# ActiveVisionLab/gaussctrl

Measured on AMD Instinct MI355X. Metric: edited views/sec @512x512 (ControlNet denoise + splat render+bwd), higher is better.
Workload: dtype bf16

## Files before the change

gaussctrl_amd/csrc/dn_gemm.hip:

```cpp
#include "dn_gemm_kernels.h"

namespace {

int choose_splits(int64_t blocks, int nk)
{
    if (blocks >= 128 || nk < 32) return 1;
    int s = (int)((448 + blocks - 1) / blocks);
    if (s > nk / 8) s = nk / 8;
    if (s > 16) s = 16;
    return s < 2 ? 1 : s;
}

int choose_mt(int64_t M, int64_t N, int ntw, bool forced)
{
    const int64_t nbn = (N + 32 * ntw - 1) / (32 * ntw);
    if (((M + 127) / 128) * nbn < 96 && !forced) return 0;
    int best = 2;
    int64_t best_cost = -1;
    for (int mt = 2; mt <= 4; ++mt) {
        const int64_t tiles = ((M + 64 * mt - 1) / (64 * mt)) * nbn;
        const int64_t cost = ((tiles + 255) / 256) * (mt + 1);
        if (best_cost < 0 || cost < best_cost || (cost == best_cost && mt == 4)) { best = mt; best_cost = cost; }
    }
    return best;
// ... 4 lines not shown
    int64_t r = total_wgs / 8 < 1 ? 1 : total_wgs / 8;
    if (r > conc) r = conc;
    const int64_t tiles = nbm * nbn;
    if (r >= tiles) return 0;
    const int64_t ca = conv ? bm : 9 * bm, cw = 9 * bn;
    int best = 0;
    int64_t best_cost = -1;
    for (int64_t pw = nbn; pw >= 1; --pw) {
        const int64_t per = nbm * pw;
        const int64_t cols = std::min<int64_t>(nbn, pw * ((r + per - 1) / per)), rows = std::min<int64_t>(nbm, (r + pw - 1) / pw);
        const int64_t cost = rows * ca + cols * cw;
        if (best_cost < 0 || cost < best_cost) { best = pw == nbn ? 0 : (int)pw; best_cost = cost; }
    }
    return best;
}

int pw_of(const gc_gemm_desc *d, int64_t nbm, int64_t nbn, int64_t total_wgs, int conc, int64_t bm, int64_t bn)
{
    const int f = (d->kernel_variant >> 16) & 0xff;
    if (f) return f - 1;
    return choose_pw(nbm, nbn, total_wgs, conc, bm, bn, d->mode == 1);
}

void plan(const gc_gemm_desc *d, int *ntw, int *splits, int *tps)
{
    *ntw = (d->N % 160 == 0 && d->N % 128 != 0 && !d->geglu) ? 5 : 4;
    if (d->softmax_keys > 0) *ntw = 5;
    const int bn = 32 * *ntw;
    const int64_t Msel = d->plan_rows > 0 ? d->plan_rows : d->M;
    const int64_t blocks = ((Msel + BM - 1) / BM) * ((d->N + bn - 1) / bn);
    const int nk = (int)((d->K + BK - 1) / BK);
    *splits = (d->geglu || d->w_set_rows > 0 || d->softmax_keys > 0) ? 1 : choose_splits(blocks, nk);
    *tps = (nk + *splits - 1) / *splits;
    *splits = (nk + *tps - 1) / *tps;
}


struct SelQ { int ntw, mt, splits, tps; };
void select_fp8(const gc_gemm_desc *d, SelQ *o, bool assume_ws)
{
    const int force_mt = d->kernel_variant & 7;
    o->ntw = (d->N % 160 == 0 && d->N % 128 != 0 && !d->geglu) ? 5 : 4;
    int mt = force_mt ? force_mt : choose_mt(d->M, d->N, o->ntw, true);
    if (o->ntw == 5) mt = 2; else if (mt > 3) mt = 3;
    if (mt < 2) mt = 2;
    const int nkq = (int)(d->K / 128);
    o->splits = 1; o->tps = nkq;
    const bool plain = !d->geglu && !d->out_t && !d->out_fp8 && !d->out_f32 && d->out && !d->ln_row_stats && !d->out_row_stats && !d->out_group_stats && d->act == 0;
    const int64_t Msel = d->plan_rows > 0 ? d->plan_rows : d->M;
    const int64_t nbn = (d->N + 32 * o->ntw - 1) / (32 * o->ntw), tiles = ((Msel + 127) / 128) * nbn;
    if (plain && !force_mt && !(d->kernel_variant & 0x40) && tiles <= 128 && nkq >= 16) {
        int s = (int)std::min<int64_t>(tiles < 96 ? (256 + tiles - 1) / tiles : 256 / tiles, nkq / 8);
        if (s > 16) s = 16;
        if (s >= 2 && (assume_ws || (d->workspace && d->workspace_bytes >= sizeof(float) * (size_t)s * (size_t)d->M * (size_t)d->N))) {
            mt = 2; o->tps = (nkq + s - 1) / s; o->splits = (nkq + o->tps - 1) / o->tps;
        }
    }
    o->mt = mt;
}
}

extern "C" size_t gc_dn_gemm_workspace_bytes(const gc_gemm_desc *d)
{
    if (!d || d->M <= 0 || d->N <= 0 || d->K <= 0) return 0;
    if (d->fp8) {
        if (d->K % 128 != 0) return 0;
        SelQ q;
        select_fp8(d, &q, true);
        return q.splits > 1 ? sizeof(float) * (size_t)q.splits * (size_t)d->M * (size_t)d->N : 0;
    }
    int ntw, splits, tps;
    plan(d, &ntw, &splits, &tps);
    return splits > 1 ? sizeof(float) * (size_t)splits * (size_t)d->M * (size_t)d->N : 0;
}

namespace {
int ln_lean_kind(const gc_gemm_desc *d)
{
    if ((d->kernel_variant & 0x800) || d->fp8 || d->mode != 0 || d->K % 64 != 0 || d->out_group_stats || d->out_chan_parts || d->N < 4) return 0;
    if (d->out_row_stats && !d->ln_row_stats)
        return (!d->geglu && d->act == 0 && !d->out_f32 && !d->out_t && d->out && (!d->rowvec || d->rows_per_batch >= 256)) ? 1 : 0;
    if (d->ln_row_stats && !d->out_row_stats) return d->softmax_keys > 0 ? 3 : 2;
    return 0;
}
struct Sel { int mode, ntw, splits, tps, mt8; };
int select(const gc_gemm_desc *d, Sel *o, bool want_parts)
{
    int mode = 0;
    if (d->mode == 1) mode = (d->Cin % 64 == 0) ? 2 : 1;
    int ntw, splits, tps;
    plan(d, &ntw, &splits, &tps);
    if (splits > 1 && (!d->workspace || d->workspace_bytes < sizeof(float) * (size_t)splits * (size_t)d->M * (size_t)d->N)) {
        splits = 1; tps = (int)((d->K + BK - 1) / BK);
    }
    const int bn = 32 * ntw;
    const int64_t nbn = (d->N + bn - 1) / bn;
    const int nk_host = (int)((d->K + BK - 1) / BK);
    const int kv = d->kernel_variant;
    const int force_mt = kv & 7;
    const int use8 = (kv & 0x10) ? 0 : ((kv & 0x20) ? 2 : 1);
    const int convsplit = (kv & 0x40) ? 0 : ((kv & 0x80) ? 1 : 2);
    o->mode = mode; o->ntw = ntw; o->splits = splits; o->tps = tps; o->mt8 = 0;
    if (use8 && d->zeros) {
        const int64_t Msel = d->plan_rows > 0 ? d->plan_rows : d->M;
        int mt = force_mt ? force_mt : choose_mt(Msel, d->N, ntw, use8 == 2);
        if (mt && !force_mt && Msel != d->M) mt = choose_mt(d->M, d->N, ntw, true);
        const int64_t tiles8 = ((Msel + 127) / 128) * nbn;
        const bool small = tiles8 < 96;
        if (!mt && mode == 0 && !force_mt) mt = 2;
        if (mode == 0 && !force_mt && ntw == 4 && d->K % 64 == 0 && !d->geglu && !d->out_t && !(kv & 0x100) &&
            (!(d->ln_row_stats || d->out_row_stats || d->out_group_stats) || ln_lean_kind(d)) && !want_parts) {
            const int64_t t1 = ((d->M + 63) / 64) * nbn, t2 = ((d->M + 127) / 128) * nbn;
            if (mt == 2 && t2 <= 256 && t1 <= 512 && t1 > 128 && nk_host <= 24) mt = 1;
        }
        if (d->w_set_rows > 0 && mt) {
            int pick = 0;
            const int cand[5] = {mt, 4, 3, 2, (ntw == 4 && d->softmax_keys == 0) ? 1 : 2};
            for (int c = 0; c < 5 && !pick; ++c) if (d->w_set_rows % (64 * cand[c]) == 0) pick = cand[c];
            mt = pick ? pick : mt;
        }
        const bool want_split = !force_mt && use8 != 2 && !d->geglu && d->w_set_rows == 0 && d->softmax_keys == 0 && d->workspace && tiles8 <= 128 && (mode == 0 ? (!small || nk_host >= 24) : (convsplit >= (small ? 2 : 1)));
        int s8 = 1, tps8 = nk_host;
        if (want_split) {
            const int smt = (kv >> 24) & 7;
            const bool img8 = mode != 0 && !small && d->Ho * d->Wo <= 64 && Msel % 256 == 0;
            const int mts = (smt >= 2 && smt <= 4) ? smt : (img8 ? 4 : ((mode != 0 && !small) ? 3 : 2));
            const int64_t tiles_s = ((Msel + 64 * mts - 1) / (64 * mts)) * nbn;
            s8 = (int)std::min<int64_t>(std::max<int64_t>(256 / tiles_s, 2), nk_host / 12);
            if (s8 >= 2 && d->workspace_bytes >= sizeof(float) * (size_t)s8 * (size_t)d->M * (size_t)d->N) {
                mt = mts; tps8 = (nk_host + s8 - 1) / s8; s8 = (nk_host + tps8 - 1) / tps8;
            } else s8 = 1;
        }
        if (splits > 1 && s8 == 1 && !force_mt && use8 != 2) mt = 0;
        if (mt) { o->mt8 = mt; o->splits = s8; o->tps = tps8; }
    }
    return 0;
}
}

extern "C" int gc_dn_gemm_row_stat_slots(const gc_gemm_desc *d)
{
    if (!d || d->M <= 0 || d->N <= 0 || d->K <= 0) return 0;
    if (d->fp8) { const int ntw = (d->N % 160 == 0 && d->N % 128 != 0) ? 5 : 4; return (int)((d->N + 16 * ntw - 1) / (16 * ntw)); }
    Sel sel;
    select(d, &sel, false);
    return sel.splits > 1 ? (int)((d->N / 4 + 63) / 64) : (int)((d->N + 16 * sel.ntw - 1) / (16 * sel.ntw));
}

namespace {
void chan_parts_layout(const gc_gemm_desc *d, const Sel &sel, int64_t *rows, int *nslab, int *col_tile)
{
    *rows = 0; *nslab = 0; *col_tile = 0;
    const int64_t rpb = d->rows_per_batch;
    if (d->fp8) {
        SelQ q;
        select_fp8(d, &q, false);
        if (d->K % 128 != 0 || rpb < 256 || rpb % 32 != 0 || d->M % rpb != 0 || d->gn_groups < 1 || d->N % d->gn_groups != 0) return;
        const int64_t cpg = d->N / d->gn_groups;
        if (q.splits > 1) {
            if (cpg > 64) return;
            *rows = CS_RB; *nslab = (int)(rpb / CS_RB); *col_tile = 64;
            return;
        }
        const bool lean = d->mode == 1 && !d->upsample && !d->geglu && !d->out_t && !d->out_fp8 && !d->out_f32 && d->out && d->act == 0 &&
                          !d->ln_row_stats && !d->out_row_stats && !d->out_group_stats;
        const int64_t bm = 64 * q.mt;
        if (!lean || bm > rpb || cpg > 32 * q.ntw) return;
        *rows = bm;
        *nslab = (int)(rpb % bm == 0 ? rpb / bm : (rpb + bm - 1) / bm + 1);
        *col_tile = 32 * q.ntw;
        return;
    }
    if (d->geglu || d->act != 0 || d->out_t || !d->out || d->out_f32 || d->ln_row_stats || d->out_row_stats || d->out_group_stats) return;
    if (rpb < 256 || rpb % 32 != 0 || d->M % rpb != 0) return;
    if (d->gn_groups < 1 || d->N % d->gn_groups != 0) return;
    const int64_t cpg = d->N / d->gn_groups;
    if (sel.splits > 1) {
        if (cpg > 64) return;
        *rows = CS_RB; *nslab = (int)(rpb / CS_RB); *col_tile = 64;
        return;
    }
    if (!sel.mt8) return;
    if ((d->mode == 1 && d->upsample) || (d->mode == 0 && d->K % 64 != 0)) return;
    const int64_t bm = 64 * (sel.mt8 < 2 ? 2 : sel.mt8);
    if (bm > rpb || cpg > 32 * sel.ntw) return;
    *rows = bm;
    *nslab = (int)(rpb % bm == 0 ? rpb / bm : (rpb + bm - 1) / bm + 1);
    *col_tile = 32 * sel.ntw;
}
}

extern "C" int gc_dn_gemm_chan_parts_layout(const gc_gemm_desc *d, int64_t *rows_per_slab, int *nslab, int *col_tile)
{
    GC_REQUIRE(d && rows_per_slab && nslab && col_tile, "null argument");
    *rows_per_slab = 0; *nslab = 0; *col_tile = 0;
    if (d->M <= 0 || d->N <= 0 || d->K <= 0 || d->rows_per_batch <= 0) return GC_OK;
    Sel sel;
    select(d, &sel, true);
    chan_parts_layout(d, sel, rows_per_slab, nslab, col_tile);
    return GC_OK;
}

extern "C" int gc_dn_gemm(const gc_gemm_desc *d, void *stream)
{
    GC_REQUIRE(d && d->W && d->A, "null descriptor / operand");
    GC_REQUIRE(d->M > 0 && d->N > 0 && d->K > 0, "empty problem");
    GC_REQUIRE(d->K % 8 == 0, "K must be a multiple of 8 (pad channels on the host)");
    GC_REQUIRE(d->N % 4 == 0, "N must be a multiple of 4 (pad output channels on the host)");
    GC_REQUIRE(d->dtype == DT_BF16 || d->dtype == DT_F16, "dtype must be 0 (bf16) or 1 (f16)");
    GemmArgs g;
    g.pw = 0;
    g.M = d->M; g.N = d->N; g.K = d->K; g.A = d->A; g.lda = d->lda;
    g.B = d->B; g.Hi = d->Hi; g.Wi = d->Wi; g.Cin = d->Cin; g.Ho = d->Ho; g.Wo = d->Wo; g.stride = d->stride; g.ups = d->upsample; g.pad = d->pad_lo;
    g.W = d->W; g.bias = d->bias; g.rowvec = d->rowvec; g.ld_rowvec = d->ld_rowvec;
    g.rows_per_batch = d->rows_per_batch > 0 ? d->rows_per_batch : 1;
    g.residual = d->residual; g.ldr = d->ldr; g.out_scale = d->out_scale; g.act = d->act; g.geglu = d->geglu;
    g.out = d->out; g.ldc = d->ldc; g.out_f32 = d->out_f32; g.out_t = d->out_t; g.ldt = d->ldt; g.t_batch_stride = d->t_batch_stride; g.t_col0 = d->t_col0;
    g.row_stats = d->ln_row_stats; g.row_stat_slots = d->ln_row_stat_slots > 0 ? d->ln_row_stat_slots : 1;
    g.colsum = d->ln_colsum; g.ln_eps = d->ln_eps; g.ln_inv_k = 1.f / (float)d->K;
    g.out_row_stats = d->out_row_stats; g.out_group_stats = d->out_group_stats; g.gn_groups = d->gn_groups;
    g.gn_cpg = d->gn_groups > 0 ? (int)(d->N / d->gn_groups) : 1;
    g.w_scale = (const unsigned char *)d->w_scale; g.a_scale = d->a_scale;
    g.out_fp8 = d->out_fp8; g.out_qscale = d->out_fp8 > 0 ? exp2f((float)(127 - d->out_fp8)) : 1.f;
    GC_REQUIRE(d->out_fp8 >= 0 && d->out_fp8 < 255, "out_fp8 must be 0 (off) or an E8M0 byte 1 .. 254");
    GC_REQUIRE(!d->out_fp8 || (d->fp8 && d->mode == 0 && d->out && !d->out_f32 && !d->out_t && !d->out_chan_parts && !d->ln_row_stats && !d->out_row_stats &&
                               !d->out_group_stats && d->ldc % 4 == 0),
               "out_fp8: an fp8 linear with a plain output (no fp32 / transposed output, no statistics, no LayerNorm fold), ldc % 4 == 0");
    g.dbg = (d->kernel_variant >> 8) & 0x0f;
    g.conv_korder = (d->kernel_variant & 0x1000) ? 0 : 1;
    g.w_set_rows = d->w_set_rows; g.w_set_stride = d->w_set_stride; g.sm_keys = d->softmax_keys;
    GC_REQUIRE(d->w_set_rows >= 0 && d->softmax_keys >= 0 && d->softmax_keys <= 80, "bad weight-set / softmax arguments");
    GC_REQUIRE(!d->softmax_keys || (d->ln_row_stats && d->N % 80 == 0 && d->out && !d->out_f32 && !d->out_t && !d->geglu && !d->residual && d->act == 0),
               "softmax_keys: a LayerNorm-folded linear with N % 80 == 0 and a plain 2-byte output");
    GC_REQUIRE((d->ln_row_stats == nullptr) == (d->ln_colsum == nullptr), "ln_row_stats and ln_colsum must be given together");
    GC_REQUIRE(!d->ln_row_stats || d->mode == 0, "LayerNorm folding applies to linear GEMMs");
    GC_REQUIRE(!(d->out_row_stats || d->out_group_stats) || (!d->geglu && !d->out_t && d->out), "output statistics need a plain (non-GEGLU, non-transposed) output");
    GC_REQUIRE(!d->out_group_stats || (g.rows_per_batch % 16 == 0 && d->gn_groups >= 1 && d->gn_groups <= GS_MAXG && d->N % d->gn_groups == 0),
               "out_group_stats needs rows_per_batch % 16 == 0 and 1 <= gn_groups <= 32 dividing N");
    if (d->mode == 1) {
        GC_REQUIRE(d->Cin % 8 == 0 && d->K == 9 * (int64_t)d->Cin, "conv3x3: K must be 9*Cin with Cin % 8 == 0");
        GC_REQUIRE(d->M == (int64_t)d->B * d->Ho * d->Wo, "conv3x3: M must be B*Ho*Wo");
        GC_REQUIRE(d->pad_lo == 0 || d->pad_lo == 1, "conv3x3: pad_lo must be 0 or 1");
    } else {
        GC_REQUIRE(d->lda >= d->K && d->lda % 8 == 0, "linear: lda must be >= K and a multiple of 8");
    }
    GC_REQUIRE((d->mode == 1 ? (int64_t)d->B * d->Hi * d->Wi * d->Cin : d->M * d->lda) < ((int64_t)1 << 31) && (int64_t)d->N * d->K < ((int64_t)1 << 31),
               "operand too large for 32-bit element offsets: split the batch");
    if (d->geglu) GC_REQUIRE(d->N % 32 == 0 && !d->out_t, "geglu needs N % 32 == 0");
    const int force_mt = d->kernel_variant & 7;
    GC_REQUIRE(force_mt >= 0 && force_mt <= 4, "kernel_variant: MT must be 0 .. 4");
    Sel sel;
    select(d, &sel, d->out_chan_parts != nullptr);
    g.chan_parts = d->out_chan_parts; g.cp_nslab = 0; g.cp_rows = 0;
    if (d->out_chan_parts) {
        int64_t rows; int ns, ct;
        chan_parts_layout(d, sel, &rows, &ns, &ct);
        GC_REQUIRE(rows > 0, "out_chan_parts: this problem cannot produce channel partials (see gc_dn_gemm_chan_parts_layout)");
        g.cp_nslab = ns; g.cp_rows = (int)rows;
        if (sel.mt8 == 1) sel.mt8 = 2;
    }
    if (fuse_of(g) && sel.mt8) {
        const bool upsampled = d->mode == 1 && d->upsample, ragged = d->mode == 0 && d->K % 64 != 0;
        GC_REQUIRE(!upsampled && !ragged, "row / group statistics and LayerNorm folding: not with upsample-fused convs or K % 64 != 0 linears");
    }
    hipStream_t s = gc::S(stream);
    g.zeros = d->zeros;
    if (d->fp8) {
        GC_REQUIRE(d->zeros && d->w_scale, "fp8: zeros page and per-row weight scales are required");
        GC_REQUIRE(d->K % 128 == 0, "fp8: K % 128 == 0");
        GC_REQUIRE(!(d->geglu || d->out_t) || (d->mode == 0 && !fuse_of(g)), "fp8: GEGLU / transposed output on linears with the plain epilogue only");
        GC_REQUIRE(d->mode == 0 || (d->Cin % 128 == 0 && !d->upsample), "fp8 conv: Cin (padded) % 128 == 0, no fused upsample");
        GC_REQUIRE(d->mode == 1 || d->lda % 16 == 0, "fp8 linear: lda % 16 == 0");
        GC_REQUIRE((int64_t)d->N * d->K < ((int64_t)1 << 31) && (d->mode == 1 ? (int64_t)d->B * d->Hi * d->Wi * d->Cin : d->M * d->lda) < ((int64_t)1 << 31), "fp8: 32-bit offsets");
        SelQ q;
        select_fp8(d, &q, false);
        const int ntw = q.ntw, mt = q.mt;
        g.splits = q.splits; g.tiles_per_split = q.tps; g.ws = q.splits > 1 ? (float *)d->workspace : nullptr;
        GC_REQUIRE(!d->out_chan_parts || q.splits > 1 || (d->mode == 1 && !fuse_of(g)), "fp8: channel partials come from k-sliced problems and fast convs");
        const int64_t nbn_q = (d->N + 32 * ntw - 1) / (32 * ntw), nbm_q = (d->M + 64 * mt - 1) / (64 * mt);
        const dim3 gq((unsigned)(nbm_q * nbn_q), (unsigned)q.splits);
        g.pw = pw_of(d, nbm_q, nbn_q, nbm_q * nbn_q * q.splits, 32, 64 * mt, 32 * ntw);
        dn_gemm_launch_fp8(g, d->dtype, d->mode == 1 ? 2 : 3, ntw, mt, gq, s);
        if (q.splits > 1) { if (g.chan_parts) dn_gemm_launch_splitk_epilogue_cs(g, d->dtype, s); else dn_gemm_launch_splitk_epilogue(g, d->dtype, s); }
        return gc::check_launch("gc_dn_gemm(fp8)");
    }
    g.splits = sel.splits; g.tiles_per_split = sel.tps; g.ws = (float *)d->workspace;
    const int bn = 32 * sel.ntw;
    const int64_t nbn = (d->N + bn - 1) / bn;
    g.persist = 0;
    const int lnk = (sel.mt8 && sel.splits == 1) ? ln_lean_kind(d) : 0;
    if (d->w_set_rows > 0 || d->softmax_keys > 0) {
        GC_REQUIRE(lnk != 0, "weight sets / softmax_keys need a lean LayerNorm-fold problem (K % 64 == 0 linear with ln_row_stats or out_row_stats, no forced variant)");
        GC_REQUIRE(d->w_set_rows == 0 || (d->w_set_rows % (64 * sel.mt8) == 0 && d->M % d->w_set_rows == 0), "w_set_rows must be a multiple of the row tile and divide M");
    }
    if (sel.mt8 == 4 && sel.ntw == 4 && sel.mode == 0 && sel.splits == 1 && d->K % 64 == 0 && d->K <= 64 * 24 && (!fuse_of(g) || lnk == 2) && !g.chan_parts &&
        !g.rowvec && !g.out_t && !g.out_f32 && g.out && g.act != 2 && !(d->kernel_variant & 0x200)) {
        const int64_t tiles = ((d->M + 255) / 256) * nbn;
        if (tiles > 256) g.persist = 256;
    }
    if (sel.mt8) {
        const int64_t nbm8 = (d->M + 64 * sel.mt8 - 1) / (64 * sel.mt8);
        const dim3 grid8((unsigned)(nbm8 * nbn), (unsigned)sel.splits);
        g.pw = pw_of(d, nbm8, nbn, g.persist ? 8 * 32 : nbm8 * nbn * sel.splits, sel.mt8 == 1 ? 64 : 32, 64 * sel.mt8, bn);
        if (lnk) dn_gemm_launch_ln(g, d->dtype, lnk, lean_of(g, sel.mode) && g.persist == 0, sel.ntw, sel.mt8, grid8, s);
        else if (fuse_of(g)) dn_gemm_launch_fuse(g, d->dtype, sel.mode, sel.ntw, sel.mt8 < 2 ? 2 : sel.mt8, grid8, s);
        else if (g.chan_parts && sel.splits == 1) dn_gemm_launch_cs(g, d->dtype, sel.mode, sel.ntw, sel.mt8, grid8, s);
        else if (lean_of(g, sel.mode) && g.persist == 0 && !(d->kernel_variant & 0x400)) dn_gemm_launch_lean(g, d->dtype, sel.mode, sel.ntw, sel.mt8, grid8, s);
        else dn_gemm_launch_plain(g, d->dtype, sel.mode, sel.ntw, sel.mt8, grid8, s);
    } else {
        const int64_t nbm = (d->M + BM - 1) / BM;
        const dim3 grid((unsigned)(nbm * nbn), (unsigned)sel.splits);
        g.pw = pw_of(d, nbm, nbn, nbm * nbn * sel.splits, 64, BM, bn);
        if (fuse_of(g)) dn_gemm_launch_fuse(g, d->dtype, sel.mode, sel.ntw, 0, grid, s); else dn_gemm_launch_plain(g, d->dtype, sel.mode, sel.ntw, 0, grid, s);
    }
    if (sel.splits > 1) { if (g.chan_parts) dn_gemm_launch_splitk_epilogue_cs(g, d->dtype, s); else dn_gemm_launch_splitk_epilogue(g, d->dtype, s); }
    return gc::check_launch("gc_dn_gemm");
}
```

gaussctrl_amd/csrc/dn_gemm_kernels.h:

```cpp
#pragma once
#include "dn_common.h"
#include <type_traits>

namespace dng {
struct GemmArgs {
    int64_t M, N, K;
    const void *A; int64_t lda;
    int B, Hi, Wi, Cin, Ho, Wo, stride, ups, pad;
    const void *W;
    const float *bias;
    const float *rowvec; int64_t ld_rowvec; int64_t rows_per_batch;
    const void *residual; int64_t ldr;
    float out_scale;
    int act, geglu;
    void *out; int64_t ldc; int out_f32;
    void *out_t; int64_t ldt; int64_t t_batch_stride; int64_t t_col0;
    int splits; int tiles_per_split;
    int persist;
    float *ws;
    const void *zeros;
    const float *row_stats; int row_stat_slots; const float *colsum; float ln_eps, ln_inv_k;
    float *out_row_stats;
    float *out_group_stats;
    int gn_groups, gn_cpg;
// ... 1071 lines not shown
                *reinterpret_cast<float2 *>(g.chan_parts + ((((b * g.cp_nslab + slab) * G + gg) * 2 + half) * 2)) = make_float2(s1, s2);
            }
        }
    } else {
    float4 bia[NTW], csm[LNV == 2 ? NTW : 1];
#pragma unroll
    for (int nt = 0; nt < NTW; ++nt) {
        const int64_t n = n_lane + nt * 16;
        bia[nt] = (g.bias && n < g.N) ? *reinterpret_cast<const float4 *>(g.bias + n) : make_float4(0.f, 0.f, 0.f, 0.f);
        if constexpr (LNV == 2) csm[nt] = n < g.N ? *reinterpret_cast<const float4 *>(g.colsum + n) : make_float4(0.f, 0.f, 0.f, 0.f);
    }
#pragma unroll
    for (int mt = 0; mt < MT; ++mt) {
        const int64_t m = m_base + wm * (16 * MT) + mt * 16 + fr;
        if (m >= g.M) continue;
        if constexpr (LNV == 2) {
            const float2 st = *reinterpret_cast<const float2 *>(srow + 2 * (wm * (16 * MT) + mt * 16 + fr));
            const float mean = st.x * g.ln_inv_k, rstd = rsqrtf(fmaxf(st.y * g.ln_inv_k - mean * mean, 0.f) + g.ln_eps);
#pragma unroll
            for (int nt = 0; nt < NTW; ++nt) {
                acc[nt][mt][0] = rstd * (acc[nt][mt][0] - mean * csm[nt].x); acc[nt][mt][1] = rstd * (acc[nt][mt][1] - mean * csm[nt].y);
                acc[nt][mt][2] = rstd * (acc[nt][mt][2] - mean * csm[nt].z); acc[nt][mt][3] = rstd * (acc[nt][mt][3] - mean * csm[nt].w);
            }
        }
        float4 rv[NTW];
        uint2 rs[NTW];
        const int64_t bidx = g.rowvec ? m / g.rows_per_batch : 0;
#pragma unroll
        for (int nt = 0; nt < NTW; ++nt) {
            const int64_t n = n_lane + nt * 16;
            const bool okn = n < g.N && !(!LEAN && g.geglu && (nt & 1));
            const int64_t on = (!LEAN && g.geglu) ? (n_base + wn * (16 * NTW) + nt * 16) / 2 + fc * 4 : n;
            rv[nt] = (g.rowvec && n < g.N) ? *reinterpret_cast<const float4 *>(g.rowvec + bidx * g.ld_rowvec + n) : make_float4(0.f, 0.f, 0.f, 0.f);
            rs[nt] = (g.residual && okn) ? *reinterpret_cast<const uint2 *>((const unsigned char *)g.residual + (m * g.ldr + on) * 2) : make_uint2(0u, 0u);
        }
#pragma unroll
        for (int nt = 0; nt < NTW; ++nt) {
            const int64_t n = n_lane + nt * 16;
            if (n >= g.N) continue;
            if (!LEAN && g.geglu && (nt & 1)) continue;
            float v[4] = {acc[nt][mt][0] + bia[nt].x + rv[nt].x, acc[nt][mt][1] + bia[nt].y + rv[nt].y,
                          acc[nt][mt][2] + bia[nt].z + rv[nt].z, acc[nt][mt][3] + bia[nt].w + rv[nt].w};
            int64_t on = n;
            if (!LEAN && g.geglu) {
                constexpr int NP = NTW - 1;
                const int np = nt + 1 < NTW ? nt + 1 : NP;
                v[0] *= gelu_erf(acc[np][mt][0] + bia[np].x); v[1] *= gelu_erf(acc[np][mt][1] + bia[np].y);
                v[2] *= gelu_erf(acc[np][mt][2] + bia[np].z); v[3] *= gelu_erf(acc[np][mt][3] + bia[np].w);
                on = (n_base + wn * (16 * NTW) + nt * 16) / 2 + fc * 4;
            }
            if (!LEAN && g.act == 1) {
#pragma unroll
                for (int r = 0; r < 4; ++r) v[r] = silu(v[r]);
            } else if (!LEAN && g.act == 2) {
#pragma unroll
                for (int r = 0; r < 4; ++r) v[r] = fminf(fmaxf(v[r] * 0.5f + 0.5f, 0.f), 1.f);
            }
#pragma unroll
            for (int r = 0; r < 4; ++r) v[r] *= g.out_scale;
            if (g.residual) {
                v[0] += T::to_f((unsigned short)(rs[nt].x & 0xffff)); v[1] += T::to_f((unsigned short)(rs[nt].x >> 16));
                v[2] += T::to_f((unsigned short)(rs[nt].y & 0xffff)); v[3] += T::to_f((unsigned short)(rs[nt].y >> 16));
            }
            const bool to_t = !LEAN && g.out_t && on >= g.t_col0;
            const uint2 pk = make_uint2(pack2<T>(v[0], v[1]), pack2<T>(v[2], v[3]));
            if (g.out && !(to_t && g.t_col0 > 0)) {
                if (!LEAN && g.out_f32)
                    *reinterpret_cast<float4 *>((float *)g.out + m * g.ldc + on) = make_float4(v[0], v[1], v[2], v[3]);
                else
                    *reinterpret_cast<uint2 *>((unsigned char *)g.out + (m * g.ldc + on) * 2) = pk;
            }
            if (to_t) {
                const int64_t b = m / g.rows_per_batch, tok = m - b * g.rows_per_batch;
                unsigned short *o = (unsigned short *)g.out_t + b * g.t_batch_stride + tok;
#pragma unroll
                for (int r = 0; r < 4; ++r) o[(on - g.t_col0 + r) * g.ldt] = T::from_f(v[r]);
            }
        }
    }
    }
}


template <class T, int NTW, int MT, int LNV = 0>
__global__ __launch_bounds__(512, 1) void k_gemm8p(const GemmArgs g)
{
    static_assert(LNV == 0 || LNV == 2, "persistent kernel: plain or LayerNorm-folded consumer");
    constexpr int BM = 64 * MT, BN = 32 * NTW, STAGE = BM * 128 + BN * 128, NS = 3;
    constexpr int AG = BM / 8, WG = BN / 8, AI = AG / 8, WI = (WG + 7) / 8;
    static_assert(WG % 8 == 0, "every wave issues the same number of W loads");
    constexpr int GRPW = AI + WI;
    extern __shared__ __attribute__((aligned(16))) unsigned char smem[];
    const int tid = threadIdx.x, lane = tid & 63;
    const int wid = __builtin_amdgcn_readfirstlane(tid >> 6);
    const int wm = wid >> 1, wn = wid & 1;
    const int nbn = (int)((g.N + BN - 1) / BN);
    const int64_t ntiles = ((g.M + BM - 1) / BM) * nbn;
    const int nk = (int)(g.K / BK);
    const unsigned lds0 = (unsigned)(size_t)(__attribute__((address_space(3))) unsigned char *)smem;
    float *srow = reinterpret_cast<float *>(smem + NS * STAGE);
    const int lr = lane >> 3, ls = lane & 7;
    const unsigned char *Ab = (const unsigned char *)g.A, *Wb = (const unsigned char *)g.W;
    auto tile_of = [&](int64_t d, int64_t &m_base, int64_t &n_base) __attribute__((always_inline)) {
        const int64_t xcd = d & 7, qq = ntiles >> 3, rr = ntiles & 7;
        const int64_t bid = (xcd < rr ? xcd * (qq + 1) : rr * (qq + 1) + (xcd - rr) * qq) + (d >> 3);
        int64_t mblk, nblk;
        dng::tile_coords(bid, (int)((g.M + BM - 1) / BM), nbn, g.pw, mblk, nblk);
        m_base = mblk * BM; n_base = nblk * BN;
    };
    int a_off[AI], w_off[WI];
    auto set_offsets = [&](int64_t m_base, int64_t n_base) __attribute__((always_inline)) {
#pragma unroll
        for (int i = 0; i < AI; ++i) {
            const int row = (wid + 8 * i) * 8 + lr;
            const int64_t m = m_base + row;
            a_off[i] = (int)(m < g.M ? m : g.M - 1) * (int)g.lda + (ls ^ ((row >> 1) & 7)) * 8;
        }
#pragma unroll
        for (int i = 0; i < WI; ++i) {
            const int row = (wid + 8 * i) * 8 + lr;
            const int64_t n = n_base + row;
            w_off[i] = (int)(n < g.N ? n : g.N - 1) * (int)g.K + (ls ^ ((row >> 1) & 7)) * 8;
        }
    };
    auto issue_a = [&](int kt, int stage, int i) __attribute__((always_inline)) {
        glds16_s(Ab + (size_t)kt * (BK * 2), (unsigned)(a_off[i] * 2), lds0 + stage * STAGE + (unsigned)((wid + 8 * i) * 1024));
    };
    auto issue_w = [&](int kt, int stage, int i) __attribute__((always_inline)) {
        glds16_s(Wb + (size_t)kt * (BK * 2), (unsigned)(w_off[i] * 2), lds0 + stage * STAGE + (unsigned)(BM * 128 + (wid + 8 * i) * 1024));
    };
    auto issue = [&](int kt, int stage) __attribute__((always_inline)) {
#pragma unroll
        for (int i = 0; i < AI; ++i) issue_a(kt, stage, i);
#pragma unroll
        for (int i = 0; i < WI; ++i) issue_w(kt, stage, i);
    };
    const int fr = lane & 15, fc = lane >> 4;
    const int swz = (fr >> 1) & 7;
    const int fx0 = ((fc ^ swz) << 4), fx1 = (((fc + 4) ^ swz) << 4);
    const int aw0 = BM * 128 + (wn * (16 * NTW) + fr) * 128, aa0 = (wm * (16 * MT) + fr) * 128;
    struct Frag { uint4 w[NTW], a[MT]; };
    auto load_frag = [&](Frag &f, int stage, int ks) __attribute__((always_inline)) {
        const unsigned char *sb = smem + stage * STAGE;
        const int fx = ks ? fx1 : fx0;
#pragma unroll
        for (int t = 0; t < NTW; ++t) f.w[t] = *reinterpret_cast<const uint4 *>(sb + aw0 + fx + t * 2048);
#pragma unroll
        for (int t = 0; t < MT; ++t) f.a[t] = *reinterpret_cast<const uint4 *>(sb + aa0 + fx + t * 2048);
    };
    f32x4 acc[NTW][MT];
    constexpr int NMM = NTW * MT, NPC = AI + WI;
    auto block = [&](const Frag &f, Frag &fn, int st_next, int ks_next, bool load_next, int dma_kt, int dma_stage, auto dma_tag) __attribute__((always_inline)) {
        constexpr bool DMA = decltype(dma_tag)::value;
        static_for<0, NMM>([&](auto m_) __attribute__((always_inline)) {
            constexpr int m = decltype(m_)::value, nt = m / MT, mt = m % MT;
            acc[nt][mt] = T::mfma(f.w[nt], f.a[mt], acc[nt][mt]);
            if constexpr (m == 0) {
                __builtin_amdgcn_sched_barrier(0);
                if (load_next) load_frag(fn, st_next, ks_next);
                __builtin_amdgcn_sched_barrier(0);
            } else if constexpr (DMA && m >= 2) {
                static_for<0, NPC>([&](auto p_) __attribute__((always_inline)) {
                    constexpr int pp = decltype(p_)::value;
                    if constexpr (m == 2 + (pp * (NMM - 3)) / NPC) {
                        __builtin_amdgcn_sched_barrier(0);
                        if constexpr (pp < AI) issue_a(dma_kt, dma_stage, pp); else issue_w(dma_kt, dma_stage, pp - AI);
                        __builtin_amdgcn_sched_barrier(0);
                    }
                });
            }
        });
    };
    auto wait_tiles = [&](auto n_) __attribute__((always_inline)) {
        asm volatile("s_waitcnt vmcnt(%0)" ::"n"(decltype(n_)::value * GRPW) : "memory");
    };

    int64_t d = blockIdx.x, m_base, n_base;
    if (d >= ntiles) return;
    tile_of(d, m_base, n_base);
    set_offsets(m_base, n_base);
    issue(0, 0);
    if (nk > 1) issue(1, 1);
    if (nk > 2) issue(2, 2);
    bool first = true;
    for (;;) {
#pragma unroll
        for (int a = 0; a < NTW; ++a)
#pragma unroll
            for (int b = 0; b < MT; ++b) acc[a][b] = f32x4{0.f, 0.f, 0.f, 0.f};
        if (first) { if (nk > 2) wait_tiles(std::integral_constant<int, 2>{}); else if (nk > 1) wait_tiles(std::integral_constant<int, 1>{}); else wait_tiles(std::integral_constant<int, 0>{}); }
        else asm volatile("s_waitcnt vmcnt(0)" ::: "memory");
        first = false;
        __builtin_amdgcn_s_barrier();
        Frag f0, f1;
        load_frag(f0, 0, 0);
        int st = 0, kt = 0;
        for (; kt + 3 < nk; ++kt) {
            const int st1 = st + 1 == NS ? 0 : st + 1;
            block(f0, f1, st, 1, true, 0, 0, std::false_type{});
            wait_tiles(std::integral_constant<int, 1>{});
            asm volatile("s_waitcnt lgkmcnt(0)" ::: "memory");
            __builtin_amdgcn_s_barrier();
            block(f1, f0, st1, 0, true, kt + 3, st, std::true_type{});
            st = st1;
        }
        for (; kt < nk; ++kt) {
            const int st1 = st + 1 == NS ? 0 : st + 1;
            block(f0, f1, st, 1, true, 0, 0, std::false_type{});
            if (kt + 1 < nk) {
                if (kt + 2 < nk) wait_tiles(std::integral_constant<int, 1>{}); else wait_tiles(std::integral_constant<int, 0>{});
                asm volatile("s_waitcnt lgkmcnt(0)" ::: "memory");
                __builtin_amdgcn_s_barrier();
                block(f1, f0, st1, 0, true, 0, 0, std::false_type{});
            } else {
                block(f1, f0, st1, 0, false, 0, 0, std::false_type{});
            }
            st = st1;
        }
        const int64_t cm = m_base, cn = n_base;
        d += gridDim.x;
        const bool more = d < ntiles;
        asm volatile("s_waitcnt lgkmcnt(0)" ::: "memory");
        __builtin_amdgcn_s_barrier();
        if constexpr (LNV == 2) {
            row_stats_prologue<BM>(g, cm, srow);
            __builtin_amdgcn_s_barrier();
        }
        if (more) {
            tile_of(d, m_base, n_base);
            set_offsets(m_base, n_base);
            issue(0, 0);
            if (nk > 1) issue(1, 1);
            if (nk > 2) issue(2, 2);
        }
        {
            const int64_t n_lane = cn + wn * (16 * NTW) + fc * 4;
            float4 bia[NTW], csm[LNV == 2 ? NTW : 1];
#pragma unroll
            for (int nt = 0; nt < NTW; ++nt) {
                const int64_t n = n_lane + nt * 16;
                bia[nt] = (g.bias && n < g.N) ? *reinterpret_cast<const float4 *>(g.bias + n) : make_float4(0.f, 0.f, 0.f, 0.f);
                if constexpr (LNV == 2) csm[nt] = n < g.N ? *reinterpret_cast<const float4 *>(g.colsum + n) : make_float4(0.f, 0.f, 0.f, 0.f);
            }
            float2 st[LNV == 2 ? MT : 1];
            if constexpr (LNV == 2) {
#pragma unroll
                for (int mt = 0; mt < MT; ++mt) st[mt] = *reinterpret_cast<const float2 *>(srow + 2 * (wm * (16 * MT) + mt * 16 + fr));
            }
#pragma unroll
            for (int mt = 0; mt < MT; ++mt) {
                const int64_t m = cm + wm * (16 * MT) + mt * 16 + fr;
                if (m >= g.M) continue;
                if constexpr (LNV == 2) {
                    const float mean = st[mt].x * g.ln_inv_k, rstd = rsqrtf(fmaxf(st[mt].y * g.ln_inv_k - mean * mean, 0.f) + g.ln_eps);
#pragma unroll
                    for (int nt = 0; nt < NTW; ++nt) {
                        acc[nt][mt][0] = rstd * (acc[nt][mt][0] - mean * csm[nt].x); acc[nt][mt][1] = rstd * (acc[nt][mt][1] - mean * csm[nt].y);
                        acc[nt][mt][2] = rstd * (acc[nt][mt][2] - mean * csm[nt].z); acc[nt][mt][3] = rstd * (acc[nt][mt][3] - mean * csm[nt].w);
                    }
                }
#pragma unroll
                for (int nt = 0; nt < NTW; ++nt) {
                    const int64_t n = n_lane + nt * 16;
                    if (n >= g.N) continue;
                    if (g.geglu && (nt & 1)) continue;
                    float v[4] = {acc[nt][mt][0] + bia[nt].x, acc[nt][mt][1] + bia[nt].y, acc[nt][mt][2] + bia[nt].z, acc[nt][mt][3] + bia[nt].w};
                    int64_t on = n;
                    if (g.geglu) {
                        constexpr int NP = NTW - 1;
                        const int np = nt + 1 < NTW ? nt + 1 : NP;
                        v[0] *= gelu_erf(acc[np][mt][0] + bia[np].x); v[1] *= gelu_erf(acc[np][mt][1] + bia[np].y);
                        v[2] *= gelu_erf(acc[np][mt][2] + bia[np].z); v[3] *= gelu_erf(acc[np][mt][3] + bia[np].w);
                        on = (cn + wn * (16 * NTW) + nt * 16) / 2 + fc * 4;
                    }
                    if (g.act == 1) {
#pragma unroll
                        for (int r = 0; r < 4; ++r) v[r] = silu(v[r]);
                    }
#pragma unroll
                    for (int r = 0; r < 4; ++r) v[r] *= g.out_scale;
                    if (g.residual) {
                        const uint2 rs = *reinterpret_cast<const uint2 *>((const unsigned char *)g.residual + (m * g.ldr + on) * 2);
                        v[0] += T::to_f((unsigned short)(rs.x & 0xffff)); v[1] += T::to_f((unsigned short)(rs.x >> 16));
                        v[2] += T::to_f((unsigned short)(rs.y & 0xffff)); v[3] += T::to_f((unsigned short)(rs.y >> 16));
                    }
                    *reinterpret_cast<uint2 *>((unsigned char *)g.out + (m * g.ldc + on) * 2) = make_uint2(pack2<T>(v[0], v[1]), pack2<T>(v[2], v[3]));
                }
            }
        }
        if (!more) break;
    }
}

template <class T, int NTW, int MT, int LNV = 0>
void launch8p(const GemmArgs &g, int nwg, hipStream_t s)
{
    constexpr size_t lds = 3 * (64 * MT * 128 + 32 * NTW * 128) + (LNV == 2 ? 64 * MT * 8 : 0);
    static_assert(lds <= 160 * 1024, "LDS ring");
    static gc::AttrOnce once;
    gc::ensure_dynamic_lds(once, (const void *)k_gemm8p<T, NTW, MT, LNV>, (int)lds);
    hipLaunchKernelGGL((k_gemm8p<T, NTW, MT, LNV>), dim3(nwg), dim3(512), lds, s, g);
}

typedef __attribute__((ext_vector_type(8))) int i32x8;

template <class T, int MODE, int NTW, int MT, bool FUSE, bool CS = false>
__global__ __launch_bounds__(512, 1) void k_gemm8q(const GemmArgs g)
{
    static_assert(MODE == 2 || MODE == 3, "fp8 path: fast conv (2) and aligned linear (3)");
    constexpr int BM = 64 * MT, BN = 32 * NTW, STAGE = BM * 128 + BN * 128, NS = 3;
    constexpr int AG = BM / 8, WG = BN / 8, AI = AG / 8, WI = (WG + 7) / 8;
    constexpr int BKB = 128;
    extern __shared__ __attribute__((aligned(16))) unsigned char smem[];
    const int tid = threadIdx.x, lane = tid & 63;
    const int wid = __builtin_amdgcn_readfirstlane(tid >> 6);
    const int wm = wid >> 1, wn = wid & 1;
    const int nbn = (int)((g.N + BN - 1) / BN);
    int64_t mblk, nblk;
    int slice;
    wg_tile(g, (int)((g.M + BM - 1) / BM), nbn, mblk, nblk, slice);
    const int64_t m_base = mblk * BM, n_base = nblk * BN;
    const int nk_all = (int)(g.K / BKB);
    const int k0 = g.splits > 1 ? slice * g.tiles_per_split : 0;
    const int nk = g.splits > 1 ? (nk_all - k0 < g.tiles_per_split ? nk_all - k0 : g.tiles_per_split) : nk_all;
    const unsigned lds0 = (unsigned)(size_t)(__attribute__((address_space(3))) unsigned char *)smem;
    float *srow = reinterpret_cast<float *>(smem + NS * STAGE);
    if constexpr (FUSE) {
        if (g.row_stats) row_stats_prologue<BM>(g, m_base, srow);
    }
    static_assert(!(FUSE && CS), "one statistics epilogue at a time");
    float *ctab = reinterpret_cast<float *>(smem + NS * STAGE);
    if constexpr (CS) {
        for (int i = tid; i < 4 * BN; i += 512) ctab[i] = 0.f;
    }
    const int lr = lane >> 3, ls = lane & 7;
    int a_off[AI];
    unsigned a_vm[AI];
    const unsigned char *a_ptr[AI];
#pragma unroll
    for (int i = 0; i < AI; ++i) {
        const int row = (wid + 8 * i) * 8 + lr;
        const int ck = ls ^ ((row >> 1) & 7);
        const int64_t m = m_base + row;
        const bool ok = m < g.M;
        a_vm[i] = 0; a_ptr[i] = (const unsigned char *)g.A; a_off[i] = 0;
        if (MODE == 2) {
            const int mm = ok ? (int)m : 0, hw = g.Ho * g.Wo, b = mm / hw, rem = mm - b * hw, oy = rem / g.Wo;
            const int y0 = oy * g.stride - g.pad, x0 = (rem - oy * g.Wo) * g.stride - g.pad;
            a_ptr[i] = (const unsigned char *)g.A + ((int64_t)(b * g.Hi + y0) * g.Wi + x0) * g.Cin + ck * 16;
            unsigned vm = 0;
#pragma unroll
            for (int tp = 0; tp < 9; ++tp) {
                const int yi = y0 + tp / 3, xi = x0 + tp % 3;
                if (ok && (unsigned)yi < (unsigned)g.Hi && (unsigned)xi < (unsigned)g.Wi) vm |= 1u << tp;
            }
            a_vm[i] = vm;
        } else {
            a_off[i] = (int)(m < g.M ? m : g.M - 1) * (int)g.lda + ck * 16;
        }
    }
    int w_off[WI];
#pragma unroll
    for (int i = 0; i < WI; ++i) {
        const int row = (wid + 8 * i) * 8 + lr;
        const int64_t n = n_base + row;
        w_off[i] = (int)(n < g.N ? n : g.N - 1) * (int)g.K + (ls ^ ((row >> 1) & 7)) * 16;
    }
    const unsigned char *Ab = (const unsigned char *)g.A, *Wb = (const unsigned char *)g.W, *Zp = (const unsigned char *)g.zeros;
    const bool tap_inner = MODE == 2 && g.conv_korder != 0;
    int ld_tap = 0, ld_ci = 0;
    if (MODE == 2) {
        if (tap_inner) { ld_tap = k0 % 9; ld_ci = (k0 / 9) * BKB; }
        else { ld_tap = (k0 * BKB) / g.Cin; ld_ci = (k0 * BKB) % g.Cin; }
    }
    struct TileSrc { int kb, tap, tap_off; unsigned sbase; };
    auto issue_begin = [&](int kt, int stage) __attribute__((always_inline)) -> TileSrc {
        TileSrc t;
        t.kb = (k0 + kt) * BKB; t.tap = 0; t.tap_off = 0;
        if (MODE == 2) {
            t.tap = ld_tap;
// ... 451 lines not shown
                }
        }
#pragma unroll
        for (int i = 0; i < RPT; ++i) {
            const int64_t m = m0 + rl + 16 * i;
            if (m >= g.M) break;
            float gate[4] = {0.f, 0.f, 0.f, 0.f};
            epilogue_store<T>(g, m, n, n, v[i], gate, &rpre[i]);
#pragma unroll
            for (int r = 0; r < 4; ++r) { cs[2 * r] += v[i][r]; cs[2 * r + 1] += v[i][r] * v[i][r]; }
        }
    }
#pragma unroll
    for (int j = 0; j < 8; ++j) red[rl][cl][j] = cs[j];
    __syncthreads();
    __shared__ float chs[64][2];
    if (threadIdx.x < 128) {
        const int c2 = threadIdx.x >> 3, j = threadIdx.x & 7;
        float o = 0.f;
#pragma unroll
        for (int r = 0; r < 16; ++r) o += red[r][c2][j];
        chs[c2 * 4 + (j >> 1)][j & 1] = o;
    }
    __syncthreads();
    if (m0 < g.M) {
        const int cpg = g.gn_cpg, G = (int)(g.N / cpg);
        const int n_base = (int)blockIdx.x * 64, n_hi = n_base + 64 < (int)g.N ? n_base + 64 : (int)g.N;
        const int g_first = n_base / cpg, ng = (n_hi - 1) / cpg - g_first + 1;
        if ((int)threadIdx.x < ng) {
            const int gg = g_first + threadIdx.x;
            const int c_lo = gg * cpg > n_base ? gg * cpg : n_base, c_hi = (gg + 1) * cpg < n_hi ? (gg + 1) * cpg : n_hi;
            float s1 = 0.f, s2 = 0.f;
            for (int c = c_lo; c < c_hi; ++c) { s1 += chs[c - n_base][0]; s2 += chs[c - n_base][1]; }
            const int64_t b = m0 / g.rows_per_batch, slab = (m0 - b * g.rows_per_batch) / CS_RB;
            const int half = gg * cpg < n_base ? 1 : 0;
            *reinterpret_cast<float2 *>(g.chan_parts + ((((b * g.cp_nslab + slab) * G + gg) * 2 + half) * 2)) = make_float2(s1, s2);
        }
    }
}


inline bool fuse_of(const GemmArgs &g) { return g.row_stats || g.out_row_stats || g.out_group_stats; }

template <class T, int MODE, int NTW, bool FUSE>
void launch4(const GemmArgs &g, dim3 grid, hipStream_t s)
{
    constexpr size_t lds = 2 * (BM * 128 + 32 * NTW * 128);
    static gc::AttrOnce once;
    gc::ensure_dynamic_lds(once, (const void *)k_gemm<T, MODE, NTW, FUSE>, (int)lds);
    hipLaunchKernelGGL((k_gemm<T, MODE, NTW, FUSE>), grid, dim3(NT), lds, s, g);
}

template <class T, int MODE, int NTW, int MT, bool FUSE, bool CS = false, bool LEAN = false, int LNV = 0>
void launch8(const GemmArgs &g, dim3 grid, hipStream_t s)
{
    constexpr size_t lds = 3 * (64 * MT * 128 + 32 * NTW * 128) + ((FUSE || LNV >= 2) ? 64 * MT * 8 : 0) + (CS ? 32 * NTW * 16 : 0);
    static_assert(lds <= 160 * 1024, "LDS ring");
    static gc::AttrOnce once;
    gc::ensure_dynamic_lds(once, (const void *)k_gemm8<T, MODE, NTW, MT, FUSE, CS, LEAN, LNV>, (int)lds);
    hipLaunchKernelGGL((k_gemm8<T, MODE, NTW, MT, FUSE, CS, LEAN, LNV>), grid, dim3(512), lds, s, g);
}

inline bool ln_lean_producer_of(const GemmArgs &g, int mode, int splits)
{
    return g.out_row_stats && !g.row_stats && !g.out_group_stats && !g.chan_parts && splits == 1 && mode == 0 && g.K % 64 == 0 && !g.geglu &&
           g.act == 0 && !g.out_f32 && !g.out_t && g.out && g.N >= 4 && (!g.rowvec || g.rows_per_batch >= 256);
}
inline bool ln_lean_consumer_of(const GemmArgs &g, int mode, int splits)
{
    return g.row_stats && !g.out_row_stats && !g.out_group_stats && !g.chan_parts && splits == 1 && mode == 0 && g.K % 64 == 0 && g.N >= 4;
}
template <class T, int NTW, int MT>
void dispatch8ln_m(const GemmArgs &g, int lnv, bool lean, dim3 grid, hipStream_t s)
{
    if (lnv == 3) { if constexpr (NTW == 5) launch8<T, 3, 5, MT, false, false, false, 3>(g, grid, s); return; }
    if (lnv == 1) launch8<T, 3, NTW, MT, false, false, true, 1>(g, grid, s);
    else if (lean) launch8<T, 3, NTW, MT, false, false, true, 2>(g, grid, s);
    else launch8<T, 3, NTW, MT, false, false, false, 2>(g, grid, s);
}
template <class T>
void dispatch8ln(const GemmArgs &g, int lnv, bool lean, int ntw, int mt, dim3 grid, hipStream_t s)
{
    if (lnv == 2 && g.persist > 0 && ntw == 4 && mt == 4) { launch8p<T, 4, 4, 2>(g, g.persist, s); return; }
    if (mt == 1 && ntw == 4) { dispatch8ln_m<T, 4, 1>(g, lnv, lean, grid, s); return; }
    if (mt < 2) mt = 2;
    if (ntw == 5) {
        if (mt == 4) dispatch8ln_m<T, 5, 4>(g, lnv, lean, grid, s); else if (mt == 3) dispatch8ln_m<T, 5, 3>(g, lnv, lean, grid, s); else dispatch8ln_m<T, 5, 2>(g, lnv, lean, grid, s);
    } else {
        if (mt == 4) dispatch8ln_m<T, 4, 4>(g, lnv, lean, grid, s); else if (mt == 3) dispatch8ln_m<T, 4, 3>(g, lnv, lean, grid, s); else dispatch8ln_m<T, 4, 2>(g, lnv, lean, grid, s);
    }
}

inline bool lean_of(const GemmArgs &g, int mode)
{
    return !g.geglu && g.act == 0 && !g.out_f32 && !g.out_t && g.out && mode != 1 && (mode != 0 || g.K % 64 == 0) && g.N >= 4 &&
           (!g.rowvec || g.rows_per_batch >= 256);
}
template <class T, int NTW, int MT>
void dispatch8lean_m(const GemmArgs &g, int mode, dim3 grid, hipStream_t s)
{
    if (mode == 0) launch8<T, 3, NTW, MT, false, false, true>(g, grid, s);
    else if (g.ups) launch8<T, 4, NTW, MT, false, false, true>(g, grid, s);
    else launch8<T, 2, NTW, MT, false, false, true>(g, grid, s);
}
template <class T>
void dispatch8lean(const GemmArgs &g, int mode, int ntw, int mt, dim3 grid, hipStream_t s)
{
    if (mt == 1 && ntw == 4 && mode == 0) { launch8<T, 3, 4, 1, false, false, true>(g, grid, s); return; }
    if (mt < 2) mt = 2;
    if (ntw == 5) {
        if (mt == 4) dispatch8lean_m<T, 5, 4>(g, mode, grid, s); else if (mt == 3) dispatch8lean_m<T, 5, 3>(g, mode, grid, s); else dispatch8lean_m<T, 5, 2>(g, mode, grid, s);
    } else {
        if (mt == 4) dispatch8lean_m<T, 4, 4>(g, mode, grid, s); else if (mt == 3) dispatch8lean_m<T, 4, 3>(g, mode, grid, s); else dispatch8lean_m<T, 4, 2>(g, mode, grid, s);
    }
}

template <class T, int NTW, int MT>
void dispatch8cs_m(const GemmArgs &g, int mode, dim3 grid, hipStream_t s)
{
    if (mode == 0) launch8<T, 3, NTW, MT, false, true>(g, grid, s);
    else if (mode == 1) launch8<T, 1, NTW, MT, false, true>(g, grid, s);
    else launch8<T, 2, NTW, MT, false, true>(g, grid, s);
}
template <class T>
void dispatch8cs(const GemmArgs &g, int mode, int ntw, int mt, dim3 grid, hipStream_t s)
{
    if (mt < 2) mt = 2;
    if (ntw == 5) {
        if (mt == 4) dispatch8cs_m<T, 5, 4>(g, mode, grid, s); else if (mt == 3) dispatch8cs_m<T, 5, 3>(g, mode, grid, s); else dispatch8cs_m<T, 5, 2>(g, mode, grid, s);
    } else {
        if (mt == 4) dispatch8cs_m<T, 4, 4>(g, mode, grid, s); else if (mt == 3) dispatch8cs_m<T, 4, 3>(g, mode, grid, s); else dispatch8cs_m<T, 4, 2>(g, mode, grid, s);
    }
}

template <class T, int NTW, int MT, bool FUSE>
void dispatch8m(const GemmArgs &g, int mode, dim3 grid, hipStream_t s)
{
    if constexpr (FUSE) {
        if (mode == 0) launch8<T, 3, NTW, MT, true>(g, grid, s);
        else if (mode == 1) launch8<T, 1, NTW, MT, true>(g, grid, s);
        else launch8<T, 2, NTW, MT, true>(g, grid, s);
    } else {
        if (mode == 0) { if (g.K % 64 == 0) launch8<T, 3, NTW, MT, false>(g, grid, s); else launch8<T, 0, NTW, MT, false>(g, grid, s); }
        else if (mode == 1) launch8<T, 1, NTW, MT, false>(g, grid, s);
        else if (g.ups) launch8<T, 4, NTW, MT, false>(g, grid, s); else launch8<T, 2, NTW, MT, false>(g, grid, s);
    }
}
template <class T, bool FUSE>
void dispatch8(const GemmArgs &g, int mode, int ntw, int mt, dim3 grid, hipStream_t s)
{
    if constexpr (!FUSE) {
        if (mt == 1 && ntw == 4 && mode == 0 && g.K % 64 == 0) { launch8<T, 3, 4, 1, false>(g, grid, s); return; }
        if (g.persist > 0 && ntw == 4 && mt == 4 && mode == 0) { launch8p<T, 4, 4>(g, g.persist, s); return; }
    }
    if (mt < 2) mt = 2;
    if (ntw == 5) {
        if (mt == 4) dispatch8m<T, 5, 4, FUSE>(g, mode, grid, s); else if (mt == 3) dispatch8m<T, 5, 3, FUSE>(g, mode, grid, s); else dispatch8m<T, 5, 2, FUSE>(g, mode, grid, s);
    } else {
        if (mt == 4) dispatch8m<T, 4, 4, FUSE>(g, mode, grid, s); else if (mt == 3) dispatch8m<T, 4, 3, FUSE>(g, mode, grid, s); else dispatch8m<T, 4, 2, FUSE>(g, mode, grid, s);
    }
}

template <class T, bool FUSE>
void dispatch4(const GemmArgs &g, int mode, int ntw, dim3 grid, hipStream_t s)
{
    if (ntw == 5) {
        if (mode == 0) launch4<T, 0, 5, FUSE>(g, grid, s); else if (mode == 1) launch4<T, 1, 5, FUSE>(g, grid, s); else launch4<T, 2, 5, FUSE>(g, grid, s);
    } else {
        if (mode == 0) launch4<T, 0, 4, FUSE>(g, grid, s); else if (mode == 1) launch4<T, 1, 4, FUSE>(g, grid, s); else launch4<T, 2, 4, FUSE>(g, grid, s);
    }
}

}

using dng::GemmArgs;
void dn_gemm_launch_plain(const GemmArgs &g, int dtype, int mode, int ntw, int mt8, dim3 grid, hipStream_t s);
void dn_gemm_launch_fuse(const GemmArgs &g, int dtype, int mode, int ntw, int mt8, dim3 grid, hipStream_t s);
void dn_gemm_launch_fp8(const GemmArgs &g, int dtype, int mode, int ntw, int mt, dim3 grid, hipStream_t s);
void dn_gemm_launch_splitk_epilogue(const GemmArgs &g, int dtype, hipStream_t s);
void dn_gemm_launch_cs(const GemmArgs &g, int dtype, int mode, int ntw, int mt8, dim3 grid, hipStream_t s);
void dn_gemm_launch_splitk_epilogue_cs(const GemmArgs &g, int dtype, hipStream_t s);
void dn_gemm_launch_lean(const GemmArgs &g, int dtype, int mode, int ntw, int mt8, dim3 grid, hipStream_t s);
void dn_gemm_launch_ln(const GemmArgs &g, int dtype, int lnv, bool lean, int ntw, int mt8, dim3 grid, hipStream_t s);
```

Before: 10.65.

## Add 192x256 persistent GEMM tile with two-stage LDS ring for wide linears

Adds a wider column tile (NTW=8, MT=3, 192x256) to the persistent bf16 GEMM kernel and selects it for large linear layers whose N is a multiple of 256, based on a tile-count cost model. To fit the larger tile in LDS, the persistent kernel's ring buffer becomes two stages when NTW>=8, and the wait counts and prefetch distance are made stage-generic. The wider tile gives more reuse of each A tile across columns, at the cost of shallower load pipelining and higher register pressure.

Result: no change. 10.67, median of 6 (+0.1%).

```diff
diff --git a/gaussctrl_amd/csrc/dn_gemm.hip b/gaussctrl_amd/csrc/dn_gemm.hip
--- a/gaussctrl_amd/csrc/dn_gemm.hip
+++ b/gaussctrl_amd/csrc/dn_gemm.hip
@@ -110,6 +110,22 @@
         return (!d->geglu && d->act == 0 && !d->out_f32 && !d->out_t && d->out && (!d->rowvec || d->rows_per_batch >= 256)) ? 1 : 0;
     if (d->ln_row_stats && !d->out_row_stats) return d->softmax_keys > 0 ? 3 : 2;
     return 0;
+}
+bool persist_legal(const gc_gemm_desc *d, int mode, int splits, bool want_parts)
+{
+    return mode == 0 && splits == 1 && d->K % 64 == 0 && d->K <= 64 * 24 && !(d->kernel_variant & 0x200) && !d->out_chan_parts && !want_parts &&
+           !d->rowvec && !d->out_t && !d->out_f32 && d->out && d->act != 2 && !d->fp8 &&
+           (!(d->ln_row_stats || d->out_row_stats || d->out_group_stats) || ln_lean_kind(d) == 2);
+}
+bool wide_legal(const gc_gemm_desc *d, int mode, int splits, bool want_parts)
+{
+    return d->N % 256 == 0 && !(d->kernel_variant & (7 | 0x800 | 0x2000)) && d->w_set_rows == 0 && d->softmax_keys == 0 &&
+           persist_legal(d, mode, splits, want_parts) && ((d->M + 191) / 192) * (d->N / 256) > 256;
+}
+int64_t tile_cost(int64_t M, int64_t N, int ntw, int mt)
+{
+    const int64_t tiles = ((M + 64 * mt - 1) / (64 * mt)) * ((N + 32 * ntw - 1) / (32 * ntw));
+    return ((tiles + 255) / 256) * (mt * ntw * (ntw == 8 ? 7 : 8) + 32);
 }
 struct Sel { int mode, ntw, splits, tps, mt8; };
 int select(const gc_gemm_desc *d, Sel *o, bool want_parts)
@@ -160,6 +176,9 @@
             } else s8 = 1;
         }
         if (splits > 1 && s8 == 1 && !force_mt && use8 != 2) mt = 0;
+        if (mt >= 2 && ntw == 4 && wide_legal(d, mode, s8, want_parts) && ((kv & 0x4000) || tile_cost(d->M, d->N, 8, 3) < tile_cost(d->M, d->N, 4, mt))) {
+            o->ntw = 8; mt = 3;
+        }
         if (mt) { o->mt8 = mt; o->splits = s8; o->tps = tps8; }
     }
     return 0;
@@ -321,11 +340,12 @@
         GC_REQUIRE(lnk != 0, "weight sets / softmax_keys need a lean LayerNorm-fold problem (K % 64 == 0 linear with ln_row_stats or out_row_stats, no forced variant)");
         GC_REQUIRE(d->w_set_rows == 0 || (d->w_set_rows % (64 * sel.mt8) == 0 && d->M % d->w_set_rows == 0), "w_set_rows must be a multiple of the row tile and divide M");
     }
-    if (sel.mt8 == 4 && sel.ntw == 4 && sel.mode == 0 && sel.splits == 1 && d->K % 64 == 0 && d->K <= 64 * 24 && (!fuse_of(g) || lnk == 2) && !g.chan_parts &&
-        !g.rowvec && !g.out_t && !g.out_f32 && g.out && g.act != 2 && !(d->kernel_variant & 0x200)) {
-        const int64_t tiles = ((d->M + 255) / 256) * nbn;
+    if (((sel.mt8 == 4 && sel.ntw == 4) || sel.ntw == 8) && sel.mode == 0 && sel.splits == 1 && d->K % 64 == 0 && d->K <= 64 * 24 && (!fuse_of(g) || lnk == 2) &&
+        !g.chan_parts && !g.rowvec && !g.out_t && !g.out_f32 && g.out && g.act != 2 && !(d->kernel_variant & 0x200)) {
+        const int64_t tiles = ((d->M + 64 * sel.mt8 - 1) / (64 * sel.mt8)) * nbn;
         if (tiles > 256) g.persist = 256;
     }
+    GC_REQUIRE(sel.ntw != 8 || g.persist > 0, "internal: the 256-wide column tile exists in the persistent kernel only");
     if (sel.mt8) {
         const int64_t nbm8 = (d->M + 64 * sel.mt8 - 1) / (64 * sel.mt8);
         const dim3 grid8((unsigned)(nbm8 * nbn), (unsigned)sel.splits);
diff --git a/gaussctrl_amd/csrc/dn_gemm_kernels.h b/gaussctrl_amd/csrc/dn_gemm_kernels.h
--- a/gaussctrl_amd/csrc/dn_gemm_kernels.h
+++ b/gaussctrl_amd/csrc/dn_gemm_kernels.h
@@ -1177,14 +1177,16 @@
 }
 
 
+template <int NTW> constexpr int ring_stages() { return NTW >= 8 ? 2 : 3; }
 template <class T, int NTW, int MT, int LNV = 0>
 __global__ __launch_bounds__(512, 1) void k_gemm8p(const GemmArgs g)
 {
     static_assert(LNV == 0 || LNV == 2, "persistent kernel: plain or LayerNorm-folded consumer");
-    constexpr int BM = 64 * MT, BN = 32 * NTW, STAGE = BM * 128 + BN * 128, NS = 3;
+    constexpr int BM = 64 * MT, BN = 32 * NTW, STAGE = BM * 128 + BN * 128, NS = ring_stages<NTW>();
     constexpr int AG = BM / 8, WG = BN / 8, AI = AG / 8, WI = (WG + 7) / 8;
     static_assert(WG % 8 == 0, "every wave issues the same number of W loads");
     constexpr int GRPW = AI + WI;
+    static_assert((NS - 1) * GRPW < 64, "vmcnt range");
     extern __shared__ __attribute__((aligned(16))) unsigned char smem[];
     const int tid = threadIdx.x, lane = tid & 63;
     const int wid = __builtin_amdgcn_readfirstlane(tid >> 6);
@@ -1276,40 +1278,38 @@
     set_offsets(m_base, n_base);
     issue(0, 0);
     if (nk > 1) issue(1, 1);
-    if (nk > 2) issue(2, 2);
+    if (NS > 2 && nk > 2) issue(2, 2);
     bool first = true;
     for (;;) {
 #pragma unroll
         for (int a = 0; a < NTW; ++a)
 #pragma unroll
             for (int b = 0; b < MT; ++b) acc[a][b] = f32x4{0.f, 0.f, 0.f, 0.f};
-        if (first) { if (nk > 2) wait_tiles(std::integral_constant<int, 2>{}); else if (nk > 1) wait_tiles(std::integral_constant<int, 1>{}); else wait_tiles(std::integral_constant<int, 0>{}); }
+        if (first) { if (nk >= NS) wait_tiles(std::integral_constant<int, NS - 1>{}); else if (nk > 1) wait_tiles(std::integral_constant<int, 1>{}); else wait_tiles(std::integral_constant<int, 0>{}); }
         else asm volatile("s_waitcnt vmcnt(0)" ::: "memory");
         first = false;
         __builtin_amdgcn_s_barrier();
         Frag f0, f1;
         load_frag(f0, 0, 0);
         int st = 0, kt = 0;
-        for (; kt + 3 < nk; ++kt) {
+        for (; kt + NS < nk; ++kt) {
             const int st1 = st + 1 == NS ? 0 : st + 1;
             block(f0, f1, st, 1, true, 0, 0, std::false_type{});
-            wait_tiles(std::integral_constant<int, 1>{});
+            wait_tiles(std::integral_constant<int, NS - 2>{});
             asm volatile("s_waitcnt lgkmcnt(0)" ::: "memory");
             __builtin_amdgcn_s_barrier();
-            block(f1, f0, st1, 0, true, kt + 3, st, std::true_type{});
+            block(f1, f0, st1, 0, true, kt + NS, st, std::true_type{});
             st = st1;
         }
         for (; kt < nk; ++kt) {
             const int st1 = st + 1 == NS ? 0 : st + 1;
             block(f0, f1, st, 1, true, 0, 0, std::false_type{});
             if (kt + 1 < nk) {
-                if (kt + 2 < nk) wait_tiles(std::integral_constant<int, 1>{}); else wait_tiles(std::integral_constant<int, 0>{});
+                if (NS > 2 && kt + 2 < nk) wait_tiles(std::integral_constant<int, 1>{}); else wait_tiles(std::integral_constant<int, 0>{});
                 asm volatile("s_waitcnt lgkmcnt(0)" ::: "memory");
                 __builtin_amdgcn_s_barrier();
-                block(f1, f0, st1, 0, true, 0, 0, std::false_type{});
-            } else {
-                block(f1, f0, st1, 0, false, 0, 0, std::false_type{});
-            }
+            }
+            block(f1, f0, st1, 0, kt + 1 < nk, 0, 0, std::false_type{});
             st = st1;
         }
         const int64_t cm = m_base, cn = n_base;
@@ -1326,7 +1326,7 @@
             set_offsets(m_base, n_base);
             issue(0, 0);
             if (nk > 1) issue(1, 1);
-            if (nk > 2) issue(2, 2);
+            if (NS > 2 && nk > 2) issue(2, 2);
         }
         {
             const int64_t n_lane = cn + wn * (16 * NTW) + fc * 4;
@@ -1390,7 +1390,7 @@
 template <class T, int NTW, int MT, int LNV = 0>
 void launch8p(const GemmArgs &g, int nwg, hipStream_t s)
 {
-    constexpr size_t lds = 3 * (64 * MT * 128 + 32 * NTW * 128) + (LNV == 2 ? 64 * MT * 8 : 0);
+    constexpr size_t lds = ring_stages<NTW>() * (64 * MT * 128 + 32 * NTW * 128) + (LNV == 2 ? 64 * MT * 8 : 0);
     static_assert(lds <= 160 * 1024, "LDS ring");
     static gc::AttrOnce once;
     gc::ensure_dynamic_lds(once, (const void *)k_gemm8p<T, NTW, MT, LNV>, (int)lds);
@@ -2008,6 +2008,7 @@
 void dispatch8ln(const GemmArgs &g, int lnv, bool lean, int ntw, int mt, dim3 grid, hipStream_t s)
 {
     if (lnv == 2 && g.persist > 0 && ntw == 4 && mt == 4) { launch8p<T, 4, 4, 2>(g, g.persist, s); return; }
+    if (lnv == 2 && g.persist > 0 && ntw == 8 && mt == 3) { launch8p<T, 8, 3, 2>(g, g.persist, s); return; }
     if (mt == 1 && ntw == 4) { dispatch8ln_m<T, 4, 1>(g, lnv, lean, grid, s); return; }
     if (mt < 2) mt = 2;
     if (ntw == 5) {
@@ -2078,6 +2079,7 @@
     if constexpr (!FUSE) {
         if (mt == 1 && ntw == 4 && mode == 0 && g.K % 64 == 0) { launch8<T, 3, 4, 1, false>(g, grid, s); return; }
         if (g.persist > 0 && ntw == 4 && mt == 4 && mode == 0) { launch8p<T, 4, 4>(g, g.persist, s); return; }
+        if (g.persist > 0 && ntw == 8 && mt == 3 && mode == 0) { launch8p<T, 8, 3>(g, g.persist, s); return; }
     }
     if (mt < 2) mt = 2;
     if (ntw == 5) {
```
